# sanweiliti/RoHM

Measured on NVIDIA H100. Metric: denoised motion clips/sec (145-frame, 1000-step PoseNet p_sample_loop), higher is better.
Workload: dtype f32 (fp16 hi/lo error-compensated tensor-core GEMMs)

## Files before the change

### rohm_b200/csrc/attention.cu

```cuda
#include "attention.cuh"

#include <cmath>

#include "common.h"
#include "gemm.cuh"
#include "ptx.cuh"

namespace rohm {
namespace {

__device__ __forceinline__ float4 load_qkv4(const float* qkv, const float* qkv_lo, int f16, int64_t idx) {
  if (!f16) return *reinterpret_cast<const float4*>(qkv + idx);
  const uint2 h = *reinterpret_cast<const uint2*>(reinterpret_cast<const __half*>(qkv) + idx);
  const uint2 l = *reinterpret_cast<const uint2*>(reinterpret_cast<const __half*>(qkv_lo) + idx);
  const __half2 h0 = *reinterpret_cast<const __half2*>(&h.x), h1 = *reinterpret_cast<const __half2*>(&h.y);
  const __half2 l0 = *reinterpret_cast<const __half2*>(&l.x), l1 = *reinterpret_cast<const __half2*>(&l.y);
  return make_float4(__low2float(h0) + __low2float(l0), __high2float(h0) + __high2float(l0),
                     __low2float(h1) + __low2float(l1), __high2float(h1) + __high2float(l1));
}
template <int DH>
__global__ void __launch_bounds__(256) attention_kernel(const float* __restrict__ qkv, const float* __restrict__ qkv_lo,
                                                        float* __restrict__ ctx_hi, float* __restrict__ ctx_lo, int S,
                                                        int D, int H, float scale, int f16) {
  constexpr int KP = DH + 4;
// ... 427 lines not shown
  mxA = fmaxf(mxA, __shfl_xor_sync(0xffffffffu, mxA, 1));
  mxA = fmaxf(mxA, __shfl_xor_sync(0xffffffffu, mxA, 2));
  mxB = fmaxf(mxB, __shfl_xor_sync(0xffffffffu, mxB, 1));
  mxB = fmaxf(mxB, __shfl_xor_sync(0xffffffffu, mxB, 2));
  float sumA = 0.0f, sumB = 0.0f;
#pragma unroll
  for (int j = 0; j < NT; ++j) {
#pragma unroll
    for (int e = 0; e < 2; ++e) {
      acc[j][e] = expf(acc[j][e] - mxA);
      acc[j][2 + e] = expf(acc[j][2 + e] - mxB);
      sumA += acc[j][e];
      sumB += acc[j][2 + e];
    }
  }
  sumA += __shfl_xor_sync(0xffffffffu, sumA, 1);
  sumA += __shfl_xor_sync(0xffffffffu, sumA, 2);
  sumB += __shfl_xor_sync(0xffffffffu, sumB, 1);
  sumB += __shfl_xor_sync(0xffffffffu, sumB, 2);
  const float invA = 1.0f / sumA, invB = 1.0f / sumB;

  uint32_t ph[NK][4], pl[NK][4];
#pragma unroll
  for (int jj = 0; jj < NK; ++jj) {
    split_f16x2(acc[2 * jj][0] * invA, acc[2 * jj][1] * invA, ph[jj][0], pl[jj][0]);
    split_f16x2(acc[2 * jj][2] * invB, acc[2 * jj][3] * invB, ph[jj][1], pl[jj][1]);
    split_f16x2(acc[2 * jj + 1][0] * invA, acc[2 * jj + 1][1] * invA, ph[jj][2], pl[jj][2]);
    split_f16x2(acc[2 * jj + 1][2] * invB, acc[2 * jj + 1][3] * invB, ph[jj][3], pl[jj][3]);
  }

  const bool okA = (r0 + g) < S, okB = (r0 + g + 8) < S;
  const int64_t oA = (base + r0 + g) * D + h * DH + 2 * t;
  const int64_t oB = oA + static_cast<int64_t>(8) * D;
  const __half* vbase = (lm < 2 ? Vh : Vl) + ((lm & 1) * 8 + lr) * P;
  constexpr int NU = 4;
#pragma unroll 1
  for (int n0 = 0; n0 < DH / 8; n0 += NU) {
    float o[NU][4];
#pragma unroll
    for (int u = 0; u < NU; ++u) o[u][0] = o[u][1] = o[u][2] = o[u][3] = 0.0f;
    const __half* vp = vbase + 8 * n0;
#pragma unroll
    for (int jj = 0; jj < NK; ++jj) {
      uint32_t bf[NU][4];
#pragma unroll
      for (int u = 0; u < NU; ++u) ldmatrix_x4_trans(bf[u], vp + 16 * jj * P + 8 * u);
#pragma unroll
      for (int u = 0; u < NU; ++u) mma_f16_16x8x16(o[u], pl[jj], bf[u][0], bf[u][1]);
#pragma unroll
      for (int u = 0; u < NU; ++u) mma_f16_16x8x16(o[u], ph[jj], bf[u][2], bf[u][3]);
#pragma unroll
      for (int u = 0; u < NU; ++u) mma_f16_16x8x16(o[u], ph[jj], bf[u][0], bf[u][1]);
    }
#pragma unroll
    for (int u = 0; u < NU; ++u) {
      const int n = n0 + u;
      uint32_t hA, lA, hB, lB;
      split_f16x2(o[u][0], o[u][1], hA, lA);
      split_f16x2(o[u][2], o[u][3], hB, lB);
      if (okA) {
        *reinterpret_cast<uint32_t*>(ctx_hi + oA + 8 * n) = hA;
        *reinterpret_cast<uint32_t*>(ctx_lo + oA + 8 * n) = lA;
      }
      if (okB) {
        *reinterpret_cast<uint32_t*>(ctx_hi + oB + 8 * n) = hB;
        *reinterpret_cast<uint32_t*>(ctx_lo + oB + 8 * n) = lB;
      }
    }
  }
}

template <int DH>
size_t attention_f16_smem_bytes(int NK) { return sizeof(__half) * 4 * 16 * NK * attn_f16_pitch<DH>(); }

struct AttnWgParams {
  CUtensorMap q_hi, q_lo;
  CUtensorMap kv_hi, kv_lo;
  __half* ctx_hi;
  __half* ctx_lo;
  int S, D, H;
  float scale;
  const int* clip_off;
  const int* clip_ids;
};
constexpr int kAwKeys = 160;
constexpr int kAwQRows = 64;
constexpr int kAwQBuf = kAwQRows * 128;
constexpr int kAwKBuf = kAwKeys * 128;
constexpr int kAwSmemBytes = 4 * kAwQBuf + 8 * kAwKBuf + 1024;

__global__ void __launch_bounds__(128, 1) attention_wgmma_kernel(const __grid_constant__ AttnWgParams p) {
  extern __shared__ uint8_t aw_smem_raw[];
  __shared__ uint64_t bar_qk, bar_v;
  const uint32_t raw = ptx::smem_u32(aw_smem_raw);
  uint8_t* const sm = aw_smem_raw + ((1024u - (raw & 1023u)) & 1023u);
  uint8_t* const Qb = sm;
  uint8_t* const Kb = sm + 4 * kAwQBuf;
  uint8_t* const Vb = Kb + 4 * kAwKBuf;
  const int qtiles = (p.S + kAwQRows - 1) / kAwQRows;
  const int qt = static_cast<int>(blockIdx.x) % qtiles;
  const int bh = static_cast<int>(blockIdx.x) / qtiles;
  const int h = bh % p.H, b = bh / p.H;
  const int q0 = qt * kAwQRows;
  int S = p.S, row0 = b * p.S;
  if (p.clip_off != nullptr) {
    const int c = p.clip_ids[b];
    row0 = p.clip_off[c];
    S = p.clip_off[c + 1] - row0;
    if (q0 >= S) return;
  }
  const int warp = threadIdx.x >> 5, lane = threadIdx.x & 31;
  if (threadIdx.x == 0) {
    ptx::prefetch_tmap(&p.q_hi);
    ptx::prefetch_tmap(&p.q_lo);
    ptx::prefetch_tmap(&p.kv_hi);
    ptx::prefetch_tmap(&p.kv_lo);
    ptx::mbar_init(&bar_qk, 1);
    ptx::mbar_init(&bar_v, 1);
    ptx::fence_barrier_init();
  }
  __syncthreads();
  ptx::pdl_launch_dependents();
  ptx::pdl_wait_prior_grid();
  if (threadIdx.x == 0) {
    ptx::mbar_expect_tx(&bar_qk, 4 * kAwQBuf + 4 * kAwKBuf);
    for (int pl = 0; pl < 2; ++pl)
      for (int c = 0; c < 2; ++c) {
        ptx::tma_load_2d(Qb + (pl * 2 + c) * kAwQBuf, pl ? &p.q_lo : &p.q_hi, &bar_qk, h * 128 + 64 * c, row0 + q0);
        ptx::tma_load_2d(Kb + (pl * 2 + c) * kAwKBuf, pl ? &p.kv_lo : &p.kv_hi, &bar_qk, p.D + h * 128 + 64 * c, row0);
      }
    ptx::mbar_expect_tx(&bar_v, 4 * kAwKBuf);
    for (int pl = 0; pl < 2; ++pl)
      for (int c = 0; c < 2; ++c)
        ptx::tma_load_2d(Vb + (pl * 2 + c) * kAwKBuf, pl ? &p.kv_lo : &p.kv_hi, &bar_v, 2 * p.D + h * 128 + 64 * c, row0);
  }

  float s[80];
#pragma unroll
  for (int i = 0; i < 80; ++i) s[i] = 0.0f;
  ptx::mbar_wait(&bar_qk, 0);
  ptx::wgmma_fence_regs(s);
  ptx::wgmma_fence();
#pragma unroll
  for (int k = 0; k < 8; ++k) {
    const int c = k >> 2;
    const uint64_t ko = static_cast<uint64_t>((k & 3) * 2);
    const uint64_t qh = ptx::make_desc_kmajor<128>(ptx::smem_u32(Qb + c * kAwQBuf)) + ko;
    const uint64_t ql = ptx::make_desc_kmajor<128>(ptx::smem_u32(Qb + (2 + c) * kAwQBuf)) + ko;
    const uint64_t kh = ptx::make_desc_kmajor<128>(ptx::smem_u32(Kb + c * kAwKBuf)) + ko;
    const uint64_t kl = ptx::make_desc_kmajor<128>(ptx::smem_u32(Kb + (2 + c) * kAwKBuf)) + ko;
    ptx::wgmma_f16(s, ql, kh);
    ptx::wgmma_f16(s, qh, kl);
    ptx::wgmma_f16(s, qh, kh);
  }
  ptx::wgmma_commit();
  ptx::wgmma_wait<0>();
  ptx::wgmma_fence_regs(s);

  const int c2 = 2 * (lane & 3);
  float m0 = -INFINITY, m1 = -INFINITY;
#pragma unroll
  for (int j = 0; j < 20; ++j) {
#pragma unroll
    for (int e = 0; e < 2; ++e) {
      const bool valid = 8 * j + c2 + e < S;
      s[4 * j + e] = valid ? s[4 * j + e] : -INFINITY;
      s[4 * j + 2 + e] = valid ? s[4 * j + 2 + e] : -INFINITY;
      m0 = fmaxf(m0, s[4 * j + e]);
      m1 = fmaxf(m1, s[4 * j + 2 + e]);
    }
  }
#pragma unroll
  for (int off = 1; off <= 2; off <<= 1) {
    m0 = fmaxf(m0, __shfl_xor_sync(0xffffffffu, m0, off));
    m1 = fmaxf(m1, __shfl_xor_sync(0xffffffffu, m1, off));
  }
  float l0 = 0.0f, l1 = 0.0f;
#pragma unroll
  for (int j = 0; j < 20; ++j) {
#pragma unroll
    for (int e = 0; e < 2; ++e) {
      const bool valid = 8 * j + c2 + e < S;
      const float p0 = valid ? expf((s[4 * j + e] - m0) * p.scale) : 0.0f;
      const float p1 = valid ? expf((s[4 * j + 2 + e] - m1) * p.scale) : 0.0f;
      s[4 * j + e] = p0, s[4 * j + 2 + e] = p1;
      l0 += p0, l1 += p1;
    }
  }
#pragma unroll
  for (int off = 1; off <= 2; off <<= 1) {
    l0 += __shfl_xor_sync(0xffffffffu, l0, off);
    l1 += __shfl_xor_sync(0xffffffffu, l1, off);
  }
  uint32_t ph[10][4], plo[10][4];
#pragma unroll
  for (int k = 0; k < 10; ++k)
#pragma unroll
    for (int i = 0; i < 4; ++i) ptx::split_f16x2(s[8 * k + 2 * i], s[8 * k + 2 * i + 1], ph[k][i], plo[k][i]);
#pragma unroll
  for (int k = 0; k < 10; ++k)
#pragma unroll
    for (int i = 0; i < 4; ++i) asm volatile("" : "+r"(ph[k][i]), "+r"(plo[k][i])::"memory");

  ptx::mbar_wait(&bar_v, 0);
  if (S < kAwKeys) {
    const int n = (kAwKeys - S) * 8;
    for (int i = threadIdx.x; i < 4 * n; i += 128) {
      const int buf = i / n, r = i - buf * n;
      *reinterpret_cast<uint4*>(Vb + buf * kAwKBuf + S * 128 + r * 16) = make_uint4(0u, 0u, 0u, 0u);
    }
    ptx::fence_proxy_async();
    __syncthreads();
  }

  float o[64];
#pragma unroll
  for (int i = 0; i < 64; ++i) o[i] = 0.0f;
  ptx::wgmma_fence_regs(o);
  ptx::wgmma_fence();
#pragma unroll
  for (int k = 0; k < 10; ++k) {
    const uint64_t vh = ptx::make_desc_mnmajor_sw128(ptx::smem_u32(Vb + k * 2048), kAwKBuf, 1024);
    const uint64_t vl = ptx::make_desc_mnmajor_sw128(ptx::smem_u32(Vb + 2 * kAwKBuf + k * 2048), kAwKBuf, 1024);
    ptx::wgmma_f16_rs_tb(o, plo[k], vh);
    ptx::wgmma_f16_rs_tb(o, ph[k], vl);
    ptx::wgmma_f16_rs_tb(o, ph[k], vh);
  }
  ptx::wgmma_commit();
  ptx::wgmma_wait<0>();
  ptx::wgmma_fence_regs(o);
#pragma unroll
  for (int k = 0; k < 10; ++k)
#pragma unroll
    for (int i = 0; i < 4; ++i) asm volatile("" : "+r"(ph[k][i]), "+r"(plo[k][i])::"memory");

  const int ra = q0 + warp * 16 + (lane >> 2), rb = ra + 8;
  const float ia = 1.0f / l0, ib = 1.0f / l1;
#pragma unroll
  for (int j = 0; j < 16; ++j) {
    const int col = h * 128 + 8 * j + c2;
    uint32_t hi, lo;
    if (ra < S) {
      ptx::split_f16x2(o[4 * j] * ia, o[4 * j + 1] * ia, hi, lo);
      const int64_t off = static_cast<int64_t>(row0 + ra) * p.D + col;
      *reinterpret_cast<uint32_t*>(p.ctx_hi + off) = hi;
      *reinterpret_cast<uint32_t*>(p.ctx_lo + off) = lo;
    }
    if (rb < S) {
      ptx::split_f16x2(o[4 * j + 2] * ib, o[4 * j + 3] * ib, hi, lo);
      const int64_t off = static_cast<int64_t>(row0 + rb) * p.D + col;
      *reinterpret_cast<uint32_t*>(p.ctx_hi + off) = hi;
      *reinterpret_cast<uint32_t*>(p.ctx_lo + off) = lo;
    }
  }
}

struct AttnStreamParams {
  CUtensorMap hi, lo;
  __half* ctx_hi;
  __half* ctx_lo;
  int S, D, H;
  float scale;
  const int* clip_off;
  const int* clip_ids;
};
constexpr int kAsBlock = 64;
constexpr int kAsBuf = kAsBlock * 128;
constexpr int kAsTile = 4 * kAsBuf;
constexpr int kAsStages = 2;
constexpr int kAsSmemBytes = (1 + 2 * kAsStages) * kAsTile + 1024;

__global__ void __launch_bounds__(128, 1) attention_wgmma_stream_kernel(const __grid_constant__ AttnStreamParams p) {
  extern __shared__ uint8_t as_smem_raw[];
  __shared__ uint64_t bar_q, bar_k[kAsStages], bar_v[kAsStages];
  const uint32_t raw = ptx::smem_u32(as_smem_raw);
  uint8_t* const sm = as_smem_raw + ((1024u - (raw & 1023u)) & 1023u);
  uint8_t* const Qb = sm;
  uint8_t* const Kb = sm + kAsTile;
  uint8_t* const Vb = Kb + kAsStages * kAsTile;
  const int qtiles = (p.S + kAsBlock - 1) / kAsBlock;
  const int qt = static_cast<int>(blockIdx.x) % qtiles;
  const int bh = static_cast<int>(blockIdx.x) / qtiles;
  const int h = bh % p.H, b = bh / p.H;
  const int q0 = qt * kAsBlock;
  int S = p.S, row0 = b * p.S;
  if (p.clip_off != nullptr) {
    const int c = p.clip_ids[b];
    row0 = p.clip_off[c];
    S = p.clip_off[c + 1] - row0;
    if (q0 >= S) return;
  }
  const int nblk = (S + kAsBlock - 1) / kAsBlock;
  const int kcol = p.D + h * 128, vcol = 2 * p.D + h * 128;
  const int warp = threadIdx.x >> 5, lane = threadIdx.x & 31;
  if (threadIdx.x == 0) {
    ptx::prefetch_tmap(&p.hi);
    ptx::prefetch_tmap(&p.lo);
    ptx::mbar_init(&bar_q, 1);
    for (int s = 0; s < kAsStages; ++s) ptx::mbar_init(&bar_k[s], 1), ptx::mbar_init(&bar_v[s], 1);
    ptx::fence_barrier_init();
  }
  __syncthreads();
  ptx::pdl_launch_dependents();
  ptx::pdl_wait_prior_grid();
  auto load_tile = [&](uint8_t* dst, uint64_t* bar, int col, int row) {
    ptx::mbar_expect_tx(bar, kAsTile);
    for (int pl = 0; pl < 2; ++pl)
      for (int c = 0; c < 2; ++c) ptx::tma_load_2d(dst + (pl * 2 + c) * kAsBuf, pl ? &p.lo : &p.hi, bar, col + 64 * c, row);
  };
  if (threadIdx.x == 0) {
    load_tile(Qb, &bar_q, h * 128, row0 + q0);
    for (int j = 0; j < kAsStages && j < nblk; ++j) {
      load_tile(Kb + j * kAsTile, &bar_k[j], kcol, row0 + j * kAsBlock);
      load_tile(Vb + j * kAsTile, &bar_v[j], vcol, row0 + j * kAsBlock);
    }
  }

  const int c2 = 2 * (lane & 3);
  float o[64];
#pragma unroll
  for (int i = 0; i < 64; ++i) o[i] = 0.0f;
  float m0 = -INFINITY, m1 = -INFINITY;
  float l0 = 0.0f, l1 = 0.0f;
  ptx::mbar_wait(&bar_q, 0);
#pragma unroll 1
  for (int j = 0; j < nblk; ++j) {
    const int st = j % kAsStages;
    const uint32_t phase = (j / kAsStages) & 1;
    uint8_t* const Ks = Kb + st * kAsTile;
    uint8_t* const Vs = Vb + st * kAsTile;
    const int kb = j * kAsBlock;

    float s[32];
#pragma unroll
    for (int i = 0; i < 32; ++i) s[i] = 0.0f;
// ... 110 lines not shown
      *reinterpret_cast<uint32_t*>(p.ctx_hi + off) = hi;
      *reinterpret_cast<uint32_t*>(p.ctx_lo + off) = lo;
    }
    if (rb < S) {
      ptx::split_f16x2(o[4 * j + 2] * ib, o[4 * j + 3] * ib, hi, lo);
      const int64_t off = static_cast<int64_t>(row0 + rb) * p.D + col;
      *reinterpret_cast<uint32_t*>(p.ctx_hi + off) = hi;
      *reinterpret_cast<uint32_t*>(p.ctx_lo + off) = lo;
    }
  }
}

size_t attention_mma_smem_bytes(int NT) { return sizeof(float) * 2 * 8 * NT * kAttnPitch; }

template <int DH, int NT>
cudaError_t launch_attention_mma(const AttnArgs& a, cudaStream_t st, bool pdl) {
  auto kern = attention_mma_kernel<DH, NT>;
  static bool attr_set = false;
  const size_t smem = attention_mma_smem_bytes(NT);
  if (!attr_set) {
    cudaError_t e = cudaFuncSetAttribute(kern, cudaFuncAttributeMaxDynamicSharedMemorySize, static_cast<int>(smem));
    if (e != cudaSuccess) return e;
    attr_set = true;
  }
  const int warps = (a.S + 15) / 16;
  return launch_chain(kern, dim3(a.B * a.H), dim3(32 * warps), smem, st, pdl, static_cast<const float*>(a.qkv_hi),
                      static_cast<float*>(a.ctx_hi), static_cast<float*>(a.ctx_lo), a.S, a.D, a.H, a.scale,
                      a.kind == kKindF16 ? 1 : 0);
}

template <int DH, int NK>
cudaError_t launch_attention_f16(const AttnArgs& a, cudaStream_t st, bool pdl) {
  const int warps = (a.S + 15) / 16;
  return launch_chain(attention_f16_kernel<DH, NK>, dim3(a.B * a.H), dim3(32 * warps), attention_f16_smem_bytes<DH>(NK), st,
                      pdl, static_cast<const __half*>(a.qkv_hi), static_cast<const __half*>(a.qkv_lo),
                      static_cast<__half*>(a.ctx_hi), static_cast<__half*>(a.ctx_lo), a.S, a.D, a.H, a.scale);
}

}

size_t attention_smem_bytes(int S, int DH) {
  const int Sp = (S + 31) & ~31;
  return sizeof(float) * (static_cast<size_t>(S) * (DH + 4) + static_cast<size_t>(S) * DH + 8 * DH + 8 * Sp);
}

int attention_wgmma_maps(AttnWgmmaMaps* maps, const AttnArgs& a) {
  const int D = a.D;
  int rc = make_tile_tmap_f16_sw128(&maps->q_hi, a.qkv_hi, a.rows, 3 * D, 3 * D, kAwQRows);
  if (rc == 0) rc = make_tile_tmap_f16_sw128(&maps->q_lo, a.qkv_lo, a.rows, 3 * D, 3 * D, kAwQRows);
  if (rc == 0) rc = make_tile_tmap_f16_sw128(&maps->kv_hi, a.qkv_hi, a.rows, 3 * D, 3 * D, kAwKeys);
  if (rc == 0) rc = make_tile_tmap_f16_sw128(&maps->kv_lo, a.qkv_lo, a.rows, 3 * D, 3 * D, kAwKeys);
  return rc;
}

cudaError_t attention_init_attributes(int max_tokens, int dh) {
  cudaError_t ea = cudaSuccess;
  auto set = [&](auto kern, size_t bytes) {
    if (ea == cudaSuccess) ea = cudaFuncSetAttribute(kern, cudaFuncAttributeMaxDynamicSharedMemorySize, static_cast<int>(bytes));
  };
  set(attention_mma_kernel<128, 4>, attention_mma_smem_bytes(4));
  set(attention_mma_kernel<128, 8>, attention_mma_smem_bytes(8));
  set(attention_mma_kernel<128, 12>, attention_mma_smem_bytes(12));
  set(attention_mma_kernel<128, 16>, attention_mma_smem_bytes(16));
  set(attention_mma_kernel<128, 20>, attention_mma_smem_bytes(20));
  set(attention_mma_kernel<64, 8>, attention_mma_smem_bytes(8));
  set(attention_mma_kernel<64, 20>, attention_mma_smem_bytes(20));
  set(attention_f16_kernel<128, 2>, attention_f16_smem_bytes<128>(2));
  set(attention_f16_kernel<128, 4>, attention_f16_smem_bytes<128>(4));
  set(attention_f16_kernel<128, 6>, attention_f16_smem_bytes<128>(6));
  set(attention_f16_kernel<128, 8>, attention_f16_smem_bytes<128>(8));
  set(attention_f16_kernel<128, 10>, attention_f16_smem_bytes<128>(10));
  set(attention_f16_kernel<64, 4>, attention_f16_smem_bytes<64>(4));
  set(attention_f16_kernel<64, 10>, attention_f16_smem_bytes<64>(10));
  set(attention_wgmma_kernel, kAwSmemBytes);
  set(attention_wgmma_stream_kernel, kAsSmemBytes);
  if (dh != 64 && dh != 128) return ea == cudaSuccess ? cudaErrorInvalidValue : ea;
  int simt_tokens = max_tokens < kAttnSimtMaxTokens ? max_tokens : kAttnSimtMaxTokens;
  while (simt_tokens > 1 && attention_smem_bytes(simt_tokens, dh) > kAttnSmemLimit) --simt_tokens;
  if (dh == 128) set(attention_kernel<128>, attention_smem_bytes(simt_tokens, 128));
  else set(attention_kernel<64>, attention_smem_bytes(simt_tokens, 64));
  return ea;
}

cudaError_t launch_attention(const AttnArgs& a, int which, const AttnWgmmaMaps* wg, cudaStream_t st, bool pdl) {
  const bool packed = a.clip_off != nullptr;
  if (a.B <= 0 || a.S <= 0 || a.H <= 0 || a.D % a.H != 0 || (packed ? a.S > a.rows : static_cast<int64_t>(a.B) * a.S > a.rows))
    return cudaErrorInvalidValue;
  if (packed && (a.clip_ids == nullptr || which == kAttnAuto)) return cudaErrorInvalidValue;
  const int dh = a.D / a.H;
  if (dh != 64 && dh != 128) return cudaErrorInvalidValue;
  const bool f16 = a.kind == kKindF16;
  const bool wg_ok = f16 && dh == 128 && a.S <= kAwKeys && wg != nullptr;
  const bool stream_ok = f16 && dh == 128 && wg != nullptr;
  const bool mma_ok = a.S <= kAttnWgmmaMaxTokens;
  if (which == kAttnAuto)
    which = wg_ok ? kAttnWgmma : (stream_ok && !mma_ok) ? kAttnWgmmaStream : !mma_ok ? kAttnSimt : f16 ? kAttnMmaF16 : kAttnMmaTf32;
  const int S = a.S;
  if (which == kAttnWgmmaStream) {
    if (!stream_ok) return cudaErrorInvalidValue;
    AttnStreamParams prm;
    prm.hi = wg->q_hi, prm.lo = wg->q_lo;
    prm.ctx_hi = static_cast<__half*>(a.ctx_hi), prm.ctx_lo = static_cast<__half*>(a.ctx_lo);
    prm.S = S, prm.D = a.D, prm.H = a.H, prm.scale = a.scale;
    prm.clip_off = a.clip_off, prm.clip_ids = a.clip_ids;
    const int qtiles = (S + kAsBlock - 1) / kAsBlock;
    return launch_chain(attention_wgmma_stream_kernel, dim3(a.B * a.H * qtiles), dim3(128), kAsSmemBytes, st, pdl, prm);
  }
  if (which == kAttnWgmma) {
    if (!wg_ok) return cudaErrorInvalidValue;
    AttnWgParams prm;
    prm.q_hi = wg->q_hi, prm.q_lo = wg->q_lo, prm.kv_hi = wg->kv_hi, prm.kv_lo = wg->kv_lo;
    prm.ctx_hi = static_cast<__half*>(a.ctx_hi), prm.ctx_lo = static_cast<__half*>(a.ctx_lo);
    prm.S = S, prm.D = a.D, prm.H = a.H, prm.scale = a.scale;
    prm.clip_off = a.clip_off, prm.clip_ids = a.clip_ids;
    const int qtiles = (S + kAwQRows - 1) / kAwQRows;
    return launch_chain(attention_wgmma_kernel, dim3(a.B * a.H * qtiles), dim3(128), kAwSmemBytes, st, pdl, prm);
  }
  if (packed) return cudaErrorInvalidValue;
  if (which == kAttnMmaF16) {
    if (!f16 || !mma_ok) return cudaErrorInvalidValue;
    const int nk = (S + 15) / 16;
    if (dh == 128 && nk <= 2) return launch_attention_f16<128, 2>(a, st, pdl);
    if (dh == 128 && nk <= 4) return launch_attention_f16<128, 4>(a, st, pdl);
    if (dh == 128 && nk <= 6) return launch_attention_f16<128, 6>(a, st, pdl);
    if (dh == 128 && nk <= 8) return launch_attention_f16<128, 8>(a, st, pdl);
    if (dh == 128) return launch_attention_f16<128, 10>(a, st, pdl);
    if (nk <= 4) return launch_attention_f16<64, 4>(a, st, pdl);
    return launch_attention_f16<64, 10>(a, st, pdl);
  }
  if (which == kAttnMmaTf32) {
    if (f16 || !mma_ok) return cudaErrorInvalidValue;
    const int nt = (S + 7) / 8;
    if (dh == 128 && nt <= 4) return launch_attention_mma<128, 4>(a, st, pdl);
    if (dh == 128 && nt <= 8) return launch_attention_mma<128, 8>(a, st, pdl);
    if (dh == 128 && nt <= 12) return launch_attention_mma<128, 12>(a, st, pdl);
    if (dh == 128 && nt <= 16) return launch_attention_mma<128, 16>(a, st, pdl);
    if (dh == 128) return launch_attention_mma<128, 20>(a, st, pdl);
    if (nt <= 8) return launch_attention_mma<64, 8>(a, st, pdl);
    return launch_attention_mma<64, 20>(a, st, pdl);
  }
  if (which == kAttnSimt) {
    const size_t smem = attention_smem_bytes(S, dh);
    if (S > kAttnSimtMaxTokens || smem > kAttnSmemLimit) return cudaErrorInvalidValue;
    auto kern = dh == 128 ? attention_kernel<128> : attention_kernel<64>;
    return launch_chain(kern, dim3(a.B * a.H), dim3(256), smem, st, pdl, static_cast<const float*>(a.qkv_hi),
                        static_cast<const float*>(a.qkv_lo), static_cast<float*>(a.ctx_hi), static_cast<float*>(a.ctx_lo), S,
                        a.D, a.H, a.scale, f16 ? 1 : 0);
  }
  return cudaErrorInvalidValue;
}

}
```

### rohm_b200/csrc/attention.cuh

```cuda
#pragma once
#include <cstddef>
#include <cstdint>
#include <cuda.h>
#include <cuda_runtime.h>

namespace rohm {

enum AttnKernel : int { kAttnAuto = 0, kAttnWgmma = 1, kAttnMmaF16 = 2, kAttnMmaTf32 = 3, kAttnSimt = 4, kAttnWgmmaStream = 5 };

constexpr int kAttnWgmmaMaxTokens = 160;
constexpr int kAttnSimtMaxTokens = 256;
constexpr size_t kAttnSmemLimit = 227 * 1024;

struct AttnWgmmaMaps {
  CUtensorMap q_hi, q_lo;
  CUtensorMap kv_hi, kv_lo;
};

struct AttnArgs {
  const void* qkv_hi;
  const void* qkv_lo;
  int64_t rows;
  void* ctx_hi;
  void* ctx_lo;
  int B, S, D, H;
  float scale;
  int kind;
  const int* clip_off = nullptr;
  const int* clip_ids = nullptr;
};

int attention_wgmma_maps(AttnWgmmaMaps* maps, const AttnArgs& a);

cudaError_t launch_attention(const AttnArgs& a, int which, const AttnWgmmaMaps* wg, cudaStream_t stream, bool pdl);

cudaError_t attention_init_attributes(int max_tokens, int dh);

size_t attention_smem_bytes(int S, int DH);

}
```

### rohm_b200/csrc/ptx.cuh

```cuda
#pragma once
#include <cstdint>
#include <cuda.h>
#include <cuda_fp16.h>
#include <cuda_runtime.h>

namespace rohm {
namespace ptx {

__device__ __forceinline__ uint32_t smem_u32(const void* p) {
  return static_cast<uint32_t>(__cvta_generic_to_shared(p));
}

__device__ __forceinline__ bool elect_one() {
  uint32_t pred = 0;
  asm volatile(
      "{\n\t"
      ".reg .pred P;\n\t"
      "elect.sync _|P, 0xffffffff;\n\t"
      "selp.u32 %0, 1, 0, P;\n\t"
      "}\n"
      : "=r"(pred));
  return pred != 0;
}

// ... 67 lines not shown
__device__ __forceinline__ void bulk_wait_all() { asm volatile("cp.async.bulk.wait_group 0;" ::: "memory"); }

__device__ __forceinline__ void wgmma_fence() { asm volatile("wgmma.fence.sync.aligned;" ::: "memory"); }
__device__ __forceinline__ void wgmma_commit() { asm volatile("wgmma.commit_group.sync.aligned;" ::: "memory"); }
template <int N>
__device__ __forceinline__ void wgmma_wait() {
  asm volatile("wgmma.wait_group.sync.aligned %0;" ::"n"(N) : "memory");
}
template <int R>
__device__ __forceinline__ void wgmma_fence_regs(float (&d)[R]) {
#pragma unroll
  for (int i = 0; i < R; ++i) asm volatile("" : "+f"(d[i])::"memory");
}
template <int R>
__device__ __forceinline__ void setmaxnreg_dec() {
  asm volatile("setmaxnreg.dec.sync.aligned.u32 %0;" ::"n"(R));
}
template <int R>
__device__ __forceinline__ void setmaxnreg_inc() {
  asm volatile("setmaxnreg.inc.sync.aligned.u32 %0;" ::"n"(R));
}
template <int kRowBytes>
__device__ __forceinline__ uint64_t make_desc_kmajor(uint32_t smem_addr) {
  static_assert(kRowBytes == 128 || kRowBytes == 64, "row = one swizzle span");
  uint64_t d = 0;
  d |= static_cast<uint64_t>((smem_addr & 0x3FFFFu) >> 4);
  d |= static_cast<uint64_t>(1) << 16;
  d |= static_cast<uint64_t>((8 * kRowBytes) >> 4) << 32;
  d |= static_cast<uint64_t>(kRowBytes == 128 ? 1 : 2) << 62;
  return d;
}

__device__ __forceinline__ uint64_t make_desc_mnmajor_sw128(uint32_t smem_addr, uint32_t lbo_bytes, uint32_t sbo_bytes) {
  uint64_t d = 0;
  d |= static_cast<uint64_t>((smem_addr & 0x3FFFFu) >> 4);
  d |= static_cast<uint64_t>((lbo_bytes >> 4) & 0x3FFFu) << 16;
  d |= static_cast<uint64_t>((sbo_bytes >> 4) & 0x3FFFu) << 32;
  d |= static_cast<uint64_t>(1) << 62;
  return d;
}

#define ROHM_R16_0 "%0, %1, %2, %3, %4, %5, %6, %7, %8, %9, %10, %11, %12, %13, %14, %15"
#define ROHM_R16_1 "%16, %17, %18, %19, %20, %21, %22, %23, %24, %25, %26, %27, %28, %29, %30, %31"
#define ROHM_R16_2 "%32, %33, %34, %35, %36, %37, %38, %39, %40, %41, %42, %43, %44, %45, %46, %47"
#define ROHM_R16_3 "%48, %49, %50, %51, %52, %53, %54, %55, %56, %57, %58, %59, %60, %61, %62, %63"
#define ROHM_R16_4 "%64, %65, %66, %67, %68, %69, %70, %71, %72, %73, %74, %75, %76, %77, %78, %79"
#define ROHM_F4(i) "+f"(d[i]), "+f"(d[i + 1]), "+f"(d[i + 2]), "+f"(d[i + 3])
#define ROHM_F16(i) ROHM_F4(i), ROHM_F4(i + 4), ROHM_F4(i + 8), ROHM_F4(i + 12)
#define ROHM_PRED(n) "{\n\t.reg .pred p;\n\tsetp.ne.b32 p, %" #n ", 0;\n\t"

#define ROHM_WGMMA_SS(KIND, INSTR, R, REGS, A, B, P, IMM, ...)                                                       \
  __device__ __forceinline__ void wgmma_##KIND(float (&d)[R], uint64_t desc_a, uint64_t desc_b) {                 \
    asm volatile(ROHM_PRED(P) INSTR " {" REGS "}, %" #A ", %" #B ", p" IMM ";\n\t}\n"                           \
                 : __VA_ARGS__                                                                                    \
                 : "l"(desc_a), "l"(desc_b), "r"(1));                                                             \
  }
ROHM_WGMMA_SS(f16, "wgmma.mma_async.sync.aligned.m64n32k16.f32.f16.f16", 16, ROHM_R16_0, 16, 17, 18, ", 1, 1, 0, 0",
              ROHM_F16(0))
ROHM_WGMMA_SS(f16, "wgmma.mma_async.sync.aligned.m64n64k16.f32.f16.f16", 32, ROHM_R16_0 ", " ROHM_R16_1, 32, 33, 34,
              ", 1, 1, 0, 0", ROHM_F16(0), ROHM_F16(16))
ROHM_WGMMA_SS(f16, "wgmma.mma_async.sync.aligned.m64n96k16.f32.f16.f16", 48,
              ROHM_R16_0 ", " ROHM_R16_1 ", " ROHM_R16_2, 48, 49, 50, ", 1, 1, 0, 0", ROHM_F16(0), ROHM_F16(16), ROHM_F16(32))
ROHM_WGMMA_SS(f16, "wgmma.mma_async.sync.aligned.m64n128k16.f32.f16.f16", 64,
              ROHM_R16_0 ", " ROHM_R16_1 ", " ROHM_R16_2 ", " ROHM_R16_3, 64, 65, 66, ", 1, 1, 0, 0", ROHM_F16(0),
              ROHM_F16(16), ROHM_F16(32), ROHM_F16(48))
ROHM_WGMMA_SS(f16, "wgmma.mma_async.sync.aligned.m64n160k16.f32.f16.f16", 80,
              ROHM_R16_0 ", " ROHM_R16_1 ", " ROHM_R16_2 ", " ROHM_R16_3 ", " ROHM_R16_4, 80, 81, 82, ", 1, 1, 0, 0",
              ROHM_F16(0), ROHM_F16(16), ROHM_F16(32), ROHM_F16(48), ROHM_F16(64))
ROHM_WGMMA_SS(tf32, "wgmma.mma_async.sync.aligned.m64n32k8.f32.tf32.tf32", 16, ROHM_R16_0, 16, 17, 18, ", 1, 1", ROHM_F16(0))
ROHM_WGMMA_SS(tf32, "wgmma.mma_async.sync.aligned.m64n64k8.f32.tf32.tf32", 32, ROHM_R16_0 ", " ROHM_R16_1, 32, 33, 34,
              ", 1, 1", ROHM_F16(0), ROHM_F16(16))
ROHM_WGMMA_SS(tf32, "wgmma.mma_async.sync.aligned.m64n96k8.f32.tf32.tf32", 48, ROHM_R16_0 ", " ROHM_R16_1 ", " ROHM_R16_2,
              48, 49, 50, ", 1, 1", ROHM_F16(0), ROHM_F16(16), ROHM_F16(32))
ROHM_WGMMA_SS(tf32, "wgmma.mma_async.sync.aligned.m64n128k8.f32.tf32.tf32", 64,
              ROHM_R16_0 ", " ROHM_R16_1 ", " ROHM_R16_2 ", " ROHM_R16_3, 64, 65, 66, ", 1, 1", ROHM_F16(0), ROHM_F16(16),
              ROHM_F16(32), ROHM_F16(48))

__device__ __forceinline__ void wgmma_f16_rs_tb(float (&d)[64], const uint32_t (&a)[4], uint64_t desc_b) {
  asm volatile(ROHM_PRED(69) "wgmma.mma_async.sync.aligned.m64n128k16.f32.f16.f16 {" ROHM_R16_0 ", " ROHM_R16_1 ", " ROHM_R16_2
               ", " ROHM_R16_3 "}, {%64, %65, %66, %67}, %68, p, 1, 1, 1;\n\t}\n"
               : ROHM_F16(0), ROHM_F16(16), ROHM_F16(32), ROHM_F16(48)
               : "r"(a[0]), "r"(a[1]), "r"(a[2]), "r"(a[3]), "l"(desc_b), "r"(1));
}

__device__ __forceinline__ float to_tf32(float x) {
  uint32_t r;
  asm("cvt.rna.tf32.f32 %0, %1;" : "=r"(r) : "f"(x));
  return __uint_as_float(r);
}

__device__ __forceinline__ void split_f16(float x, __half& hi, __half& lo) {
  uint16_t h;
  asm("cvt.rn.satfinite.f16.f32 %0, %1;" : "=h"(h) : "f"(x));
  hi = __ushort_as_half(h);
  lo = __float2half_rn(x - __half2float(hi));
}
__device__ __forceinline__ void split_f16x2(float x, float y, uint32_t& hi, uint32_t& lo) {
  asm("cvt.rn.satfinite.f16x2.f32 %0, %1, %2;" : "=r"(hi) : "f"(y), "f"(x));
  const float2 hf = __half22float2(*reinterpret_cast<const __half2*>(&hi));
  const float lx = x - hf.x, ly = y - hf.y;
  asm("cvt.rn.f16x2.f32 %0, %1, %2;" : "=r"(lo) : "f"(ly), "f"(lx));
}
__device__ __forceinline__ void split_f16x4(const float4& v, uint2& hi, uint2& lo) {
  split_f16x2(v.x, v.y, hi.x, lo.x);
  split_f16x2(v.z, v.w, hi.y, lo.y);
}

__device__ __forceinline__ void pdl_wait_prior_grid() { asm volatile("griddepcontrol.wait;" ::: "memory"); }
__device__ __forceinline__ void pdl_launch_dependents() { asm volatile("griddepcontrol.launch_dependents;" ::: "memory"); }

}
}
```

Baseline: 21.81.

## Share K/V across all query tiles of a head in one multi-warpgroup CTA

After: 22.14 (median of 6 runs). 1.01x the previous value.

```diff
diff --git a/rohm_b200/csrc/attention.cu b/rohm_b200/csrc/attention.cu
--- a/rohm_b200/csrc/attention.cu
+++ b/rohm_b200/csrc/attention.cu
@@ -533,175 +533,206 @@
   float scale;
   const int* clip_off;
   const int* clip_ids;
+  int one_tile;
 };
 constexpr int kAwKeys = 160;
 constexpr int kAwQRows = 64;
 constexpr int kAwQBuf = kAwQRows * 128;
 constexpr int kAwKBuf = kAwKeys * 128;
-constexpr int kAwSmemBytes = 4 * kAwQBuf + 8 * kAwKBuf + 1024;
-
-__global__ void __launch_bounds__(128, 1) attention_wgmma_kernel(const __grid_constant__ AttnWgParams p) {
+constexpr int kAwTiles = (kAwKeys + kAwQRows - 1) / kAwQRows;
+constexpr int kAwQSlots = 2;
+constexpr int kAwSmemBytes = kAwQSlots * 4 * kAwQBuf + 8 * kAwKBuf + 1024;
+static_assert(kAwSmemBytes <= static_cast<int>(kAttnSmemLimit), "Q slots, K and V must fit one CTA's shared memory");
+static_assert(kAwTiles <= 2 * kAwQSlots, "a slot is refilled once");
+
+__global__ void __launch_bounds__(128 * kAwTiles, 1) attention_wgmma_kernel(const __grid_constant__ AttnWgParams p) {
   extern __shared__ uint8_t aw_smem_raw[];
-  __shared__ uint64_t bar_qk, bar_v;
+  __shared__ uint64_t bar_k, bar_v, bar_q[kAwTiles];
   const uint32_t raw = ptx::smem_u32(aw_smem_raw);
   uint8_t* const sm = aw_smem_raw + ((1024u - (raw & 1023u)) & 1023u);
   uint8_t* const Qb = sm;
-  uint8_t* const Kb = sm + 4 * kAwQBuf;
+  uint8_t* const Kb = sm + kAwQSlots * 4 * kAwQBuf;
   uint8_t* const Vb = Kb + 4 * kAwKBuf;
-  const int qtiles = (p.S + kAwQRows - 1) / kAwQRows;
-  const int qt = static_cast<int>(blockIdx.x) % qtiles;
-  const int bh = static_cast<int>(blockIdx.x) / qtiles;
+  int bh = static_cast<int>(blockIdx.x), t0 = 0;
+  if (p.one_tile) {
+    const int qtiles = (p.S + kAwQRows - 1) / kAwQRows;
+    t0 = bh % qtiles, bh /= qtiles;
+  }
   const int h = bh % p.H, b = bh / p.H;
-  const int q0 = qt * kAwQRows;
   int S = p.S, row0 = b * p.S;
   if (p.clip_off != nullptr) {
     const int c = p.clip_ids[b];
     row0 = p.clip_off[c];
     S = p.clip_off[c + 1] - row0;
-    if (q0 >= S) return;
-  }
-  const int warp = threadIdx.x >> 5, lane = threadIdx.x & 31;
+  }
+  const int qtiles = (S + kAwQRows - 1) / kAwQRows;
+  if (t0 >= qtiles) return;
+  const int ntiles = p.one_tile ? 1 : qtiles;
+  const int wg = threadIdx.x >> 7, tid = threadIdx.x & 127;
+  const int warp = tid >> 5, lane = threadIdx.x & 31;
   if (threadIdx.x == 0) {
     ptx::prefetch_tmap(&p.q_hi);
     ptx::prefetch_tmap(&p.q_lo);
     ptx::prefetch_tmap(&p.kv_hi);
     ptx::prefetch_tmap(&p.kv_lo);
-    ptx::mbar_init(&bar_qk, 1);
+    ptx::mbar_init(&bar_k, 1);
     ptx::mbar_init(&bar_v, 1);
+    for (int i = 0; i < kAwTiles; ++i) ptx::mbar_init(&bar_q[i], 1);
     ptx::fence_barrier_init();
   }
   __syncthreads();
   ptx::pdl_launch_dependents();
   ptx::pdl_wait_prior_grid();
+  auto load_q = [&](int i) {
+    ptx::mbar_expect_tx(&bar_q[i], 4 * kAwQBuf);
+    for (int pl = 0; pl < 2; ++pl)
+      for (int c = 0; c < 2; ++c)
+        ptx::tma_load_2d(Qb + ((i % kAwQSlots) * 4 + pl * 2 + c) * kAwQBuf, pl ? &p.q_lo : &p.q_hi, &bar_q[i],
+                         h * 128 + 64 * c, row0 + (t0 + i) * kAwQRows);
+  };
   if (threadIdx.x == 0) {
-    ptx::mbar_expect_tx(&bar_qk, 4 * kAwQBuf + 4 * kAwKBuf);
+    load_q(0);
+    ptx::mbar_expect_tx(&bar_k, 4 * kAwKBuf);
     for (int pl = 0; pl < 2; ++pl)
-      for (int c = 0; c < 2; ++c) {
-        ptx::tma_load_2d(Qb + (pl * 2 + c) * kAwQBuf, pl ? &p.q_lo : &p.q_hi, &bar_qk, h * 128 + 64 * c, row0 + q0);
-        ptx::tma_load_2d(Kb + (pl * 2 + c) * kAwKBuf, pl ? &p.kv_lo : &p.kv_hi, &bar_qk, p.D + h * 128 + 64 * c, row0);
-      }
+      for (int c = 0; c < 2; ++c)
+        ptx::tma_load_2d(Kb + (pl * 2 + c) * kAwKBuf, pl ? &p.kv_lo : &p.kv_hi, &bar_k, p.D + h * 128 + 64 * c, row0);
+    for (int i = 1; i < kAwQSlots && i < ntiles; ++i) load_q(i);
     ptx::mbar_expect_tx(&bar_v, 4 * kAwKBuf);
     for (int pl = 0; pl < 2; ++pl)
       for (int c = 0; c < 2; ++c)
         ptx::tma_load_2d(Vb + (pl * 2 + c) * kAwKBuf, pl ? &p.kv_lo : &p.kv_hi, &bar_v, 2 * p.D + h * 128 + 64 * c, row0);
   }
 
-  float s[80];
-#pragma unroll
-  for (int i = 0; i < 80; ++i) s[i] = 0.0f;
-  ptx::mbar_wait(&bar_qk, 0);
-  ptx::wgmma_fence_regs(s);
-  ptx::wgmma_fence();
-#pragma unroll
-  for (int k = 0; k < 8; ++k) {
-    const int c = k >> 2;
-    const uint64_t ko = static_cast<uint64_t>((k & 3) * 2);
-    const uint64_t qh = ptx::make_desc_kmajor<128>(ptx::smem_u32(Qb + c * kAwQBuf)) + ko;
-    const uint64_t ql = ptx::make_desc_kmajor<128>(ptx::smem_u32(Qb + (2 + c) * kAwQBuf)) + ko;
-    const uint64_t kh = ptx::make_desc_kmajor<128>(ptx::smem_u32(Kb + c * kAwKBuf)) + ko;
-    const uint64_t kl = ptx::make_desc_kmajor<128>(ptx::smem_u32(Kb + (2 + c) * kAwKBuf)) + ko;
-    ptx::wgmma_f16(s, ql, kh);
-    ptx::wgmma_f16(s, qh, kl);
-    ptx::wgmma_f16(s, qh, kh);
-  }
-  ptx::wgmma_commit();
-  ptx::wgmma_wait<0>();
-  ptx::wgmma_fence_regs(s);
-
+  const bool work = wg < ntiles;
+  const int tile = t0 + wg;
   const int c2 = 2 * (lane & 3);
-  float m0 = -INFINITY, m1 = -INFINITY;
-#pragma unroll
-  for (int j = 0; j < 20; ++j) {
-#pragma unroll
-    for (int e = 0; e < 2; ++e) {
-      const bool valid = 8 * j + c2 + e < S;
-      s[4 * j + e] = valid ? s[4 * j + e] : -INFINITY;
-      s[4 * j + 2 + e] = valid ? s[4 * j + 2 + e] : -INFINITY;
-      m0 = fmaxf(m0, s[4 * j + e]);
-      m1 = fmaxf(m1, s[4 * j + 2 + e]);
-    }
-  }
-#pragma unroll
-  for (int off = 1; off <= 2; off <<= 1) {
-    m0 = fmaxf(m0, __shfl_xor_sync(0xffffffffu, m0, off));
-    m1 = fmaxf(m1, __shfl_xor_sync(0xffffffffu, m1, off));
-  }
+  uint32_t ph[10][4], plo[10][4];
   float l0 = 0.0f, l1 = 0.0f;
-#pragma unroll
-  for (int j = 0; j < 20; ++j) {
-#pragma unroll
-    for (int e = 0; e < 2; ++e) {
-      const bool valid = 8 * j + c2 + e < S;
-      const float p0 = valid ? expf((s[4 * j + e] - m0) * p.scale) : 0.0f;
-      const float p1 = valid ? expf((s[4 * j + 2 + e] - m1) * p.scale) : 0.0f;
-      s[4 * j + e] = p0, s[4 * j + 2 + e] = p1;
-      l0 += p0, l1 += p1;
-    }
-  }
-#pragma unroll
-  for (int off = 1; off <= 2; off <<= 1) {
-    l0 += __shfl_xor_sync(0xffffffffu, l0, off);
-    l1 += __shfl_xor_sync(0xffffffffu, l1, off);
-  }
-  uint32_t ph[10][4], plo[10][4];
-#pragma unroll
-  for (int k = 0; k < 10; ++k)
-#pragma unroll
-    for (int i = 0; i < 4; ++i) ptx::split_f16x2(s[8 * k + 2 * i], s[8 * k + 2 * i + 1], ph[k][i], plo[k][i]);
-#pragma unroll
-  for (int k = 0; k < 10; ++k)
-#pragma unroll
-    for (int i = 0; i < 4; ++i) asm volatile("" : "+r"(ph[k][i]), "+r"(plo[k][i])::"memory");
+  if (work) {
+    uint8_t* const Qs = Qb + (wg % kAwQSlots) * 4 * kAwQBuf;
+    float s[80];
+#pragma unroll
+    for (int i = 0; i < 80; ++i) s[i] = 0.0f;
+    ptx::mbar_wait(&bar_k, 0);
+    ptx::mbar_wait(&bar_q[wg], 0);
+    ptx::wgmma_fence_regs(s);
+    ptx::wgmma_fence();
+#pragma unroll
+    for (int k = 0; k < 8; ++k) {
+      const int c = k >> 2;
+      const uint64_t ko = static_cast<uint64_t>((k & 3) * 2);
+      const uint64_t qh = ptx::make_desc_kmajor<128>(ptx::smem_u32(Qs + c * kAwQBuf)) + ko;
+      const uint64_t ql = ptx::make_desc_kmajor<128>(ptx::smem_u32(Qs + (2 + c) * kAwQBuf)) + ko;
+      const uint64_t kh = ptx::make_desc_kmajor<128>(ptx::smem_u32(Kb + c * kAwKBuf)) + ko;
+      const uint64_t kl = ptx::make_desc_kmajor<128>(ptx::smem_u32(Kb + (2 + c) * kAwKBuf)) + ko;
+      ptx::wgmma_f16(s, ql, kh);
+      ptx::wgmma_f16(s, qh, kl);
+      ptx::wgmma_f16(s, qh, kh);
+    }
+    ptx::wgmma_commit();
+    ptx::wgmma_wait<0>();
+    ptx::wgmma_fence_regs(s);
+    if (wg + kAwQSlots < ntiles) {
+      asm volatile("bar.sync %0, 128;" ::"r"(1 + wg) : "memory");
+      if (tid == 0) load_q(wg + kAwQSlots);
+    }
+
+    float m0 = -INFINITY, m1 = -INFINITY;
+#pragma unroll
+    for (int j = 0; j < 20; ++j) {
+#pragma unroll
+      for (int e = 0; e < 2; ++e) {
+        const bool valid = 8 * j + c2 + e < S;
+        s[4 * j + e] = valid ? s[4 * j + e] : -INFINITY;
+        s[4 * j + 2 + e] = valid ? s[4 * j + 2 + e] : -INFINITY;
+        m0 = fmaxf(m0, s[4 * j + e]);
+        m1 = fmaxf(m1, s[4 * j + 2 + e]);
+      }
+    }
+#pragma unroll
+    for (int off = 1; off <= 2; off <<= 1) {
+      m0 = fmaxf(m0, __shfl_xor_sync(0xffffffffu, m0, off));
+      m1 = fmaxf(m1, __shfl_xor_sync(0xffffffffu, m1, off));
+    }
+#pragma unroll
+    for (int j = 0; j < 20; ++j) {
+#pragma unroll
+      for (int e = 0; e < 2; ++e) {
+        const bool valid = 8 * j + c2 + e < S;
+        const float p0 = valid ? expf((s[4 * j + e] - m0) * p.scale) : 0.0f;
+        const float p1 = valid ? expf((s[4 * j + 2 + e] - m1) * p.scale) : 0.0f;
+        s[4 * j + e] = p0, s[4 * j + 2 + e] = p1;
+        l0 += p0, l1 += p1;
+      }
+    }
+#pragma unroll
+    for (int off = 1; off <= 2; off <<= 1) {
+      l0 += __shfl_xor_sync(0xffffffffu, l0, off);
+      l1 += __shfl_xor_sync(0xffffffffu, l1, off);
+    }
+#pragma unroll
+    for (int k = 0; k < 10; ++k)
+#pragma unroll
+      for (int i = 0; i < 4; ++i) ptx::split_f16x2(s[8 * k + 2 * i], s[8 * k + 2 * i + 1], ph[k][i], plo[k][i]);
+#pragma unroll
+    for (int k = 0; k < 10; ++k)
+#pragma unroll
+      for (int i = 0; i < 4; ++i) asm volatile("" : "+r"(ph[k][i]), "+r"(plo[k][i])::"memory");
+  }
 
   ptx::mbar_wait(&bar_v, 0);
   if (S < kAwKeys) {
     const int n = (kAwKeys - S) * 8;
-    for (int i = threadIdx.x; i < 4 * n; i += 128) {
+    for (int i = threadIdx.x; i < 4 * n; i += 128 * kAwTiles) {
       const int buf = i / n, r = i - buf * n;
       *reinterpret_cast<uint4*>(Vb + buf * kAwKBuf + S * 128 + r * 16) = make_uint4(0u, 0u, 0u, 0u);
     }
     ptx::fence_proxy_async();
     __syncthreads();
   }
-
-  float o[64];
-#pragma unroll
-  for (int i = 0; i < 64; ++i) o[i] = 0.0f;
-  ptx::wgmma_fence_regs(o);
-  ptx::wgmma_fence();
-#pragma unroll
-  for (int k = 0; k < 10; ++k) {
-    const uint64_t vh = ptx::make_desc_mnmajor_sw128(ptx::smem_u32(Vb + k * 2048), kAwKBuf, 1024);
-    const uint64_t vl = ptx::make_desc_mnmajor_sw128(ptx::smem_u32(Vb + 2 * kAwKBuf + k * 2048), kAwKBuf, 1024);
-    ptx::wgmma_f16_rs_tb(o, plo[k], vh);
-    ptx::wgmma_f16_rs_tb(o, ph[k], vl);
-    ptx::wgmma_f16_rs_tb(o, ph[k], vh);
-  }
-  ptx::wgmma_commit();
-  ptx::wgmma_wait<0>();
-  ptx::wgmma_fence_regs(o);
-#pragma unroll
-  for (int k = 0; k < 10; ++k)
-#pragma unroll
-    for (int i = 0; i < 4; ++i) asm volatile("" : "+r"(ph[k][i]), "+r"(plo[k][i])::"memory");
-
-  const int ra = q0 + warp * 16 + (lane >> 2), rb = ra + 8;
+  if (!work) return;
+
+  const int ra = tile * kAwQRows + warp * 16 + (lane >> 2), rb = ra + 8;
   const float ia = 1.0f / l0, ib = 1.0f / l1;
-#pragma unroll
-  for (int j = 0; j < 16; ++j) {
-    const int col = h * 128 + 8 * j + c2;
-    uint32_t hi, lo;
-    if (ra < S) {
-      ptx::split_f16x2(o[4 * j] * ia, o[4 * j + 1] * ia, hi, lo);
-      const int64_t off = static_cast<int64_t>(row0 + ra) * p.D + col;
-      *reinterpret_cast<uint32_t*>(p.ctx_hi + off) = hi;
-      *reinterpret_cast<uint32_t*>(p.ctx_lo + off) = lo;
-    }
-    if (rb < S) {
-      ptx::split_f16x2(o[4 * j + 2] * ib, o[4 * j + 3] * ib, hi, lo);
-      const int64_t off = static_cast<int64_t>(row0 + rb) * p.D + col;
-      *reinterpret_cast<uint32_t*>(p.ctx_hi + off) = hi;
-      *reinterpret_cast<uint32_t*>(p.ctx_lo + off) = lo;
+#pragma unroll 1
+  for (int c = 0; c < 2; ++c) {
+    float o[32];
+#pragma unroll
+    for (int i = 0; i < 32; ++i) o[i] = 0.0f;
+    ptx::wgmma_fence_regs(o);
+    ptx::wgmma_fence();
+#pragma unroll
+    for (int k = 0; k < 10; ++k) {
+      const uint64_t vh = ptx::make_desc_mnmajor_sw128(ptx::smem_u32(Vb + c * kAwKBuf + k * 2048), kAwKBuf, 1024);
+      const uint64_t vl = ptx::make_desc_mnmajor_sw128(ptx::smem_u32(Vb + (2 + c) * kAwKBuf + k * 2048), kAwKBuf, 1024);
+      ptx::wgmma_f16_rs_tb(o, plo[k], vh);
+      ptx::wgmma_f16_rs_tb(o, ph[k], vl);
+      ptx::wgmma_f16_rs_tb(o, ph[k], vh);
+    }
+    ptx::wgmma_commit();
+    ptx::wgmma_wait<0>();
+    ptx::wgmma_fence_regs(o);
+#pragma unroll
+    for (int k = 0; k < 10; ++k)
+#pragma unroll
+      for (int i = 0; i < 4; ++i) asm volatile("" : "+r"(ph[k][i]), "+r"(plo[k][i])::"memory");
+
+#pragma unroll
+    for (int j = 0; j < 8; ++j) {
+      const int col = h * 128 + 64 * c + 8 * j + c2;
+      uint32_t hi, lo;
+      if (ra < S) {
+        ptx::split_f16x2(o[4 * j] * ia, o[4 * j + 1] * ia, hi, lo);
+        const int64_t off = static_cast<int64_t>(row0 + ra) * p.D + col;
+        *reinterpret_cast<uint32_t*>(p.ctx_hi + off) = hi;
+        *reinterpret_cast<uint32_t*>(p.ctx_lo + off) = lo;
+      }
+      if (rb < S) {
+        ptx::split_f16x2(o[4 * j + 2] * ib, o[4 * j + 3] * ib, hi, lo);
+        const int64_t off = static_cast<int64_t>(row0 + rb) * p.D + col;
+        *reinterpret_cast<uint32_t*>(p.ctx_hi + off) = hi;
+        *reinterpret_cast<uint32_t*>(p.ctx_lo + off) = lo;
+      }
     }
   }
 }
@@ -978,6 +1009,19 @@
   return ea;
 }
 
+namespace {
+bool attention_wgmma_one_tile(const AttnArgs& a) {
+  static int num_sms = 0;
+  if (num_sms == 0) {
+    int dev = 0;
+    cudaGetDevice(&dev);
+    if (cudaDeviceGetAttribute(&num_sms, cudaDevAttrMultiProcessorCount, dev) != cudaSuccess || num_sms <= 0) num_sms = 132;
+  }
+  const int64_t one_tile_ctas = static_cast<int64_t>(a.B) * a.H * ((a.S + kAwQRows - 1) / kAwQRows);
+  return one_tile_ctas <= num_sms;
+}
+}
+
 cudaError_t launch_attention(const AttnArgs& a, int which, const AttnWgmmaMaps* wg, cudaStream_t st, bool pdl) {
   const bool packed = a.clip_off != nullptr;
   if (a.B <= 0 || a.S <= 0 || a.H <= 0 || a.D % a.H != 0 || (packed ? a.S > a.rows : static_cast<int64_t>(a.B) * a.S > a.rows))
@@ -1002,15 +1046,16 @@
     const int qtiles = (S + kAsBlock - 1) / kAsBlock;
     return launch_chain(attention_wgmma_stream_kernel, dim3(a.B * a.H * qtiles), dim3(128), kAsSmemBytes, st, pdl, prm);
   }
-  if (which == kAttnWgmma) {
+  if (which == kAttnWgmma || which == kAttnWgmmaAllTiles || which == kAttnWgmmaOneTile) {
     if (!wg_ok) return cudaErrorInvalidValue;
     AttnWgParams prm;
     prm.q_hi = wg->q_hi, prm.q_lo = wg->q_lo, prm.kv_hi = wg->kv_hi, prm.kv_lo = wg->kv_lo;
     prm.ctx_hi = static_cast<__half*>(a.ctx_hi), prm.ctx_lo = static_cast<__half*>(a.ctx_lo);
     prm.S = S, prm.D = a.D, prm.H = a.H, prm.scale = a.scale;
     prm.clip_off = a.clip_off, prm.clip_ids = a.clip_ids;
-    const int qtiles = (S + kAwQRows - 1) / kAwQRows;
-    return launch_chain(attention_wgmma_kernel, dim3(a.B * a.H * qtiles), dim3(128), kAwSmemBytes, st, pdl, prm);
+    prm.one_tile = which == kAttnWgmma ? (attention_wgmma_one_tile(a) ? 1 : 0) : which == kAttnWgmmaOneTile ? 1 : 0;
+    const int ctas = a.B * a.H * (prm.one_tile ? (S + kAwQRows - 1) / kAwQRows : 1);
+    return launch_chain(attention_wgmma_kernel, dim3(ctas), dim3(128 * kAwTiles), kAwSmemBytes, st, pdl, prm);
   }
   if (packed) return cudaErrorInvalidValue;
   if (which == kAttnMmaF16) {
diff --git a/rohm_b200/csrc/attention.cuh b/rohm_b200/csrc/attention.cuh
--- a/rohm_b200/csrc/attention.cuh
+++ b/rohm_b200/csrc/attention.cuh
@@ -6,7 +6,8 @@
 
 namespace rohm {
 
-enum AttnKernel : int { kAttnAuto = 0, kAttnWgmma = 1, kAttnMmaF16 = 2, kAttnMmaTf32 = 3, kAttnSimt = 4, kAttnWgmmaStream = 5 };
+enum AttnKernel : int { kAttnAuto = 0, kAttnWgmma = 1, kAttnMmaF16 = 2, kAttnMmaTf32 = 3, kAttnSimt = 4, kAttnWgmmaStream = 5,
+                        kAttnWgmmaAllTiles = 6, kAttnWgmmaOneTile = 7 };
 
 constexpr int kAttnWgmmaMaxTokens = 160;
 constexpr int kAttnSimtMaxTokens = 256;
diff --git a/rohm_b200/csrc/ptx.cuh b/rohm_b200/csrc/ptx.cuh
--- a/rohm_b200/csrc/ptx.cuh
+++ b/rohm_b200/csrc/ptx.cuh
@@ -173,6 +173,12 @@
                : ROHM_F16(0), ROHM_F16(16), ROHM_F16(32), ROHM_F16(48)
                : "r"(a[0]), "r"(a[1]), "r"(a[2]), "r"(a[3]), "l"(desc_b), "r"(1));
 }
+__device__ __forceinline__ void wgmma_f16_rs_tb(float (&d)[32], const uint32_t (&a)[4], uint64_t desc_b) {
+  asm volatile(ROHM_PRED(37) "wgmma.mma_async.sync.aligned.m64n64k16.f32.f16.f16 {" ROHM_R16_0 ", " ROHM_R16_1
+               "}, {%32, %33, %34, %35}, %36, p, 1, 1, 1;\n\t}\n"
+               : ROHM_F16(0), ROHM_F16(16)
+               : "r"(a[0]), "r"(a[1]), "r"(a[2]), "r"(a[3]), "l"(desc_b), "r"(1));
+}
 
 __device__ __forceinline__ float to_tf32(float x) {
   uint32_t r;
```
